# jankammeth/BA-path-planning

Hardware: AMD Instinct MI355X
Metric: SCP iterations/sec (N agents x K waypoints) (higher is better)
Workload: dtype f64

## Files before the change

ba-path-planning_amd/csrc/scp_qp_persist.hip:

```cpp
#include "scp_qp_persist_device.h"

#include <algorithm>
#include <cstdlib>
#include <cerrno>
#include <chrono>


namespace {
using namespace scpdev;
using namespace scp_persist;

#ifdef SCP_PHASE_PROFILE
__device__ unsigned long long scp_persist_clk[16];
#define PSTAMP(slot)                                  \
  do {                                                \
    const unsigned long long now_ = wall_clock64();   \
    pacc[slot] += now_ - plast;                       \
    plast = now_;                                     \
  } while (0)
#else
#define PSTAMP(slot) ((void)0)
#endif

constexpr int persist_apb(int D) { return D == 3 ? 4 : CB / D; }
// ... 580 lines not shown
#pragma unroll
    for (int d = 0; d < D; ++d) {
      const int64_t g = (int64_t)k * C + (int64_t)agent * D + d;
      A.x[g] = x[d];
      A.Qx[g] = qx[d];
    }
  }
  for (int e = threadIdx.x; e < ne; e += NT) {
    A.gval[ebase + e] = e_g[e];
    if (!((e_code[e] >> 16) & 1)) {
      A.zc[e_row[e]] = e_z[e];
      A.yc[e_row[e]] = e_y[e];
      if (with_dy) A.dyc[e_row[e]] = e_pp[(size_t)e * D];
    }
  }
  PSTAMP(8);
#ifdef SCP_PHASE_PROFILE
  if (blockIdx.x == gridDim.x / 2 && threadIdx.x == 0)
    for (int i = 0; i < 16; ++i) scp_persist_clk[i] = i == 15 ? (unsigned long long)steps : pacc[i];
#endif
  if (blockIdx.x == 0 && threadIdx.x == 0) {
    const int slot[NCHK] = {SL_RP, SL_NAX, SL_NZ, SL_RD, SL_NPX, SL_NATY, SL_NDY, SL_SUPP, SL_NATDY};
#pragma unroll
    for (int j = 0; j < NCHK; ++j)
      __hip_atomic_store((u64*)(A.host_scal + slot[j]), (u64)__double_as_longlong(chk[j]), __ATOMIC_RELAXED, __HIP_MEMORY_SCOPE_SYSTEM);
    __hip_atomic_store(A.host_status + 1, (unsigned)it_done, __ATOMIC_RELAXED, __HIP_MEMORY_SCOPE_SYSTEM);
    __hip_atomic_store(A.host_status + 2, n_rho, __ATOMIC_RELAXED, __HIP_MEMORY_SCOPE_SYSTEM);
    __hip_atomic_store((u64*)A.host_rho, (u64)__double_as_longlong(rho), __ATOMIC_RELAXED, __HIP_MEMORY_SCOPE_SYSTEM);
    __hip_atomic_store(A.host_status, exit_code, __ATOMIC_RELAXED, __HIP_MEMORY_SCOPE_SYSTEM);
    __hip_atomic_store(A.host_flag, A.seq, __ATOMIC_RELEASE, __HIP_MEMORY_SCOPE_SYSTEM);
  }
}

size_t persist_lds_bytes(int K, int D, int cap, int nblk) {
  const int apb = persist_apb(D);
  size_t dbl = (size_t)3 * CB * pad_col(K) + (size_t)apb * 64 * D + (size_t)NCHK * nblk + (size_t)cap * (4 * D + 4);
  size_t ints = (size_t)3 * cap + (size_t)apb * K + 1;
  return dbl * sizeof(double) + ((ints + 1) / 2 * 2) * sizeof(int);
}

}

static int persist_variant_for(const scp_qp* qp) {
  const int max_wg = std::min(qp->ctx->n_cu, SCP_PERSIST_MAX_WG);
  const int apb = persist_apb(qp->D);
  const bool fits_old = (qp->N + apb - 1) / apb <= max_wg;
  const bool fits16 = qp->D == 2 && (qp->N + 15) / 16 <= max_wg;
  const bool fits8 = (qp->N + 7) / 8 <= max_wg;
  if (qp->st.persistent == 2 && fits16) return 1;
  if (qp->st.persistent == 3 && fits8) return 2;
  if (qp->st.persistent == 4 && fits_old) return 0;
  if (qp->D == 2) return fits8 ? 2 : (fits16 ? 1 : -1);
  return fits_old ? 0 : (fits8 ? 2 : -1);
}
static int variant_apb(int variant, int D) { return variant == 1 ? 16 : (variant == 2 ? 8 : persist_apb(D)); }

bool scp_qp_persist_eligible(const scp_qp* qp) {
  if (!qp->st.persistent || qp->st.cg_iters != 1 || qp->st.use_mfma != 1) return false;
  if (qp->K > 64 || qp->nW <= 0 || qp->persist_off) return false;
  return persist_variant_for(qp) >= 0;
}

int scp_qp_cg1_persist(scp_qp* qp, int it0, int cad0, int* ran, int* code, int* it_done) {
  const QpDev& d = qp->d;
  scp_ctx* ctx = qp->ctx;
  hipStream_t s = ctx->stream;
  const scp_qp_settings& st = qp->st;
  const int K = qp->K, D = qp->D;
  const int64_t C = qp->C, nx = (int64_t)K * C;
  const int variant = persist_variant_for(qp);
  if (variant < 0) { *ran = 0; return SCP_OK; }
  const bool lean = variant >= 1;
  const int apb = variant_apb(variant, D);
  const int nblk = (qp->N + apb - 1) / apb;
  *ran = 0;
  if (!qp->cg1_ready) {
    int rc = scp_qp_cg1_prepare(qp);
    if (rc) return rc;
  }
  if (qp->persist_cap_nW == qp->nW) return SCP_OK;
  {
    const int nb = nblk + 1;
    const size_t fixed = lean ? scp_persist16_lds_bytes(K, 0, nb, D, apb) : persist_lds_bytes(K, D, 0, nb);
    const size_t per_entry = (size_t)(4 * D + 4) * sizeof(double) + (lean ? 1 : 3) * sizeof(int);
    const size_t budget_lds = 160 * 1024 - (lean ? 2048 : 1024);
    if (fixed + 64 * per_entry > budget_lds) return SCP_OK;
    qp->persist_cap = (int)((budget_lds - fixed) / per_entry / 64 * 64);
  }
  const int nblk_expected = nblk + (qp->persist_fault > 0 ? 1 : 0);
  const size_t lds = lean ? scp_persist16_lds_bytes(K, qp->persist_cap, nblk_expected, D, apb)
                          : persist_lds_bytes(K, D, qp->persist_cap, nblk_expected);
  if (lds > 160 * 1024) return SCP_OK;
  const int budget = st.max_iter - it0;
  if (budget <= 0) return SCP_OK;
  if (!scp_persist_claim(ctx->device, ctx->n_cu, nblk, 200)) {
    qp->persist_skip_solve = true;
    return SCP_OK;
  }
  if (qp->persist_fault > 0) --qp->persist_fault;
  struct ClaimGuard {
    int device, n;
    ~ClaimGuard() { scp_persist_release(device, n); }
  } claim_guard{ctx->device, nblk};
  PersistArgs a;
  a.K = K; a.N = qp->N; a.nblk = nblk_expected; a.ent_cap = qp->persist_cap;
  a.it0 = it0; a.max_iter = st.max_iter; a.check_every = st.check_termination;
  a.cad0 = cad0 > 0 ? cad0 : st.check_termination; a.fine_ratio = st.check_fine_ratio;
  a.check_fine = (st.check_fine > 0 && st.check_fine < st.check_termination && st.check_termination % st.check_fine == 0 && C <= 4096)
                     ? st.check_fine : 0;
  a.rho_interval = st.adaptive_rho_interval > 0 ? st.adaptive_rho_interval : 1;
  a.C = C;
  a.rho = qp->rho; a.rho_c = qp->rho * st.rho_col_scale; a.rho_eq = st.rho_eq_scale; a.alpha = st.alpha; a.h = qp->h;
  a.eps_abs = st.eps_abs; a.eps_rel = st.eps_rel; a.eps_prim_inf = st.eps_prim_inf;
  a.vel_lo = qp->lim[0]; a.vel_hi = qp->lim[1];
  a.acc_lo = qp->lim[2]; a.acc_hi = qp->lim[3]; a.jerk_lo = qp->lim[4]; a.jerk_hi = qp->lim[5];
  for (int dd = 0; dd < 3; ++dd) { a.pmin[dd] = qp->space[dd]; a.pmax[dd] = qp->space[3 + dd]; }
  a.states = d.states;
  a.first_step = qp->steps_since_reset == 0 ? 1 : 0;
  {
    static const int spin_sleep = [] {
      const char* e = getenv("SCP_PERSIST_SPIN_SLEEP");
      const int v = e ? atoi(e) : 1;
      return v < 1 ? 1 : (v > 64 ? 64 : v);
    }();
    a.spin_sleep = spin_sleep;
  }
  a.rho_tol = (st.adaptive_rho && st.adaptive_rho_interval > 0) ? st.adaptive_rho_tolerance : 0.0;
  a.pMinv = d.pMinv;
  a.pT = d.pT;
  a.lf = d.lf; a.uf = d.uf; a.zf = d.zf; a.yf = d.yf; a.fx = d.fx; a.x = d.x;
  a.Qx = qp->qx_sel ? d.HQ : d.HQ + nx;
  a.dyf = d.dyf;
  a.cells = d.cells;
  a.gpart = d.gpart;
  a.gcheck = d.gcheck;
  a.give_up = (unsigned*)d.sync_words;
  a.cell_ptr = d.cell_ptr; a.ent_code = d.ent_code; a.w_k = d.w_k; a.w_i = d.w_i; a.w_j = d.w_j;
  a.w_eta = d.w_eta; a.w_l = d.w_l; a.zc = d.zc; a.yc = d.yc; a.dyc = d.dyc; a.gval = d.gval;
  a.host_status = qp->h_persist_dev;
  a.host_scal = qp->h_scal_dev;
  a.host_flag = (u64*)(qp->h_scal_dev + SL_COUNT + SCP_RESID_CAP);
  a.host_rho = qp->h_scal_dev + SL_COUNT + SCP_RESID_CAP + 3;
  a.rho_col_scale = st.rho_col_scale;
  a.n_tab = 0;
  for (int i = 0; i < qp->n_kkt; ++i)
    if (qp->kkt[i].used && qp->kkt[i].sigma == st.sigma) {
      a.tab[a.n_tab].rho = qp->kkt[i].rho;
      a.tab[a.n_tab].pMinv = qp->kkt[i].pMinv;
      a.tab[a.n_tab].pT = qp->kkt[i].pT;
      ++a.n_tab;
    }
  a.seq = ++qp->check_seq;
  qp->h_persist[0] = 0u;
  qp->h_persist[1] = (unsigned)it0;
  qp->h_persist[2] = 0u;
  qp->persist_rho_switches = 0;
  if (qp->persist_epoch == 0 || qp->persist_epoch + (u64)budget >= 0x7FFFFFF0ull) {
    SCP_HIP_CHECK(ctx, hipMemsetAsync(d.sync_words, 0, 16, s));
    SCP_HIP_CHECK(ctx, hipMemsetAsync(d.cells, 0, (size_t)K * C * 2 * sizeof(u64), s));
    SCP_HIP_CHECK(ctx, hipMemsetAsync(d.gpart, 0, (size_t)SCP_GPART_WORDS * sizeof(u64), s));
    SCP_HIP_CHECK(ctx, hipMemsetAsync(d.gcheck, 0, (size_t)SCP_GCHECK_WORDS * sizeof(u64), s));
    qp->persist_epoch = 0;
  }
  a.epoch0 = (unsigned)qp->persist_epoch;
  qp->persist_variant = variant;
  if (lean) {
    int rc = scp_persist16_launch(ctx, a, nblk, lds, D, apb);
// ... 153 lines not shown
```

ba-path-planning_amd/csrc/scp_qp_persist16.hip:

```cpp
#include "scp_qp_persist_device.h"

namespace {
using namespace scpdev;
using namespace scp_persist;

#ifdef SCP_PHASE_PROFILE
__device__ unsigned long long scp_persist16_clk[16];
#define PSTAMP(slot)                                           \
  do {                                                         \
    if (prof_t) {                                              \
      const unsigned long long now_ = wall_clock64();          \
      pacc_s[slot] += now_ - pacc_s[15];                       \
      pacc_s[15] = now_;                                       \
    }                                                          \
  } while (0)
#else
#define PSTAMP(slot) ((void)0)
#endif

constexpr int nct_of(int D, int APB) { return (D * APB + 15) / 16; }
constexpr int AB_STRIDE = 32;

struct Lds16 {
  int RSK, tK, nks;
  size_t rt, pt, ml, gp, ab, gchk, ent, n_dbl;
  __host__ __device__ Lds16(int K, int cap, int nblk, int D, int APB) {
    const int NC16 = 16 * nct_of(D, APB), APB16 = APB;
    RSK = pad_col(K);
    tK = (K + 15) >> 4;
    nks = (K + 3) >> 2;
    size_t o = 0;
    rt = o; o += (size_t)NC16 * RSK;
    pt = o; o += (size_t)NC16 * RSK;
    ml = o; o += (size_t)tK * nks * 64;
    gp = o; o += (size_t)2 * nblk;
    ab = o; o += (size_t)APB16 * AB_STRIDE;
    if ((size_t)2 * NC16 * RSK >= (size_t)NCHK * nblk) gchk = rt;
    else { gchk = o; o += (size_t)NCHK * nblk; }
    ent = o; o += (size_t)cap * (4 * D + 4);
    n_dbl = o;
  }
};

template <int D, int APB16>
__global__ __launch_bounds__(64 * APB16) void cg1_persist16_kernel(PersistArgs A) {
  constexpr int NT16 = 64 * APB16;
  constexpr int NCT = nct_of(D, APB16);
  constexpr int NC16 = 16 * NCT;
  extern __shared__ __attribute__((aligned(16))) double lds[];
  __shared__ double red[NCHK][APB16];
  __shared__ double cert_s[3][APB16];
  __shared__ double chk_s[NCHK];
  __shared__ int fail_s;
#ifdef SCP_PHASE_PROFILE
  __shared__ unsigned long long pacc_s[16];
  const bool prof_t = blockIdx.x == gridDim.x / 2 && threadIdx.x == 0;
  if (prof_t) {
    for (int i = 0; i < 15; ++i) pacc_s[i] = 0;
    pacc_s[15] = wall_clock64();
  }
#endif
  const int K = A.K, N = A.N;
  const int64_t C = A.C;
  const int cap = A.ent_cap, nblk = A.nblk;
  const Lds16 L(K, cap, nblk, D, APB16);
  const int RSK = L.RSK, tK = L.tK, nks = L.nks;
  double* Rt = lds + L.rt;
  double* Pt = lds + L.pt;
  double* Ml = lds + L.ml;
  double* gp = lds + L.gp;
  double* ab = lds + L.ab;
  double* gck = lds + L.gchk;
  double* e_c = lds + L.ent;
  double* e_l = e_c + (size_t)cap * D;
  double* e_z = e_l + cap;
  double* e_y = e_z + cap;
  double* e_g = e_y + cap;
  double* e_qo = e_g + cap;
  double* e_qp = e_qo + (size_t)cap * D;
  double* e_pp = e_qp + (size_t)cap * D;
  int* e_code = (int*)(lds + L.n_dbl);
  int* cptr = e_code + cap;

  const int wave = threadIdx.x >> 6, lane = threadIdx.x & 63;
  const int a0 = blockIdx.x * APB16;
  const int agent = a0 + wave;
  const bool aok = agent < N;
  const int k = lane;
  const bool live = aok && k < K;
  const bool jok = live && k < K - 1;
  const bool lastk = k == K - 1;
  const double h = A.h, hh = h * h, ih = 1.0 / h, alpha = A.alpha;
  double rho = A.rho, rho_c = A.rho_c;
  unsigned n_rho = 0;

  const int a1 = min(a0 + APB16, N);
  const int ebase = A.cell_ptr[cell_of(0, a0, K)];
  const int ne = A.cell_ptr[cell_of(0, a1, K)] - ebase;
  {
    int worst = 0;
    for (int b = threadIdx.x; b < (N + APB16 - 1) / APB16; b += NT16) {
      const int b0 = b * APB16, b1 = min(b0 + APB16, N);
      worst = max(worst, A.cell_ptr[cell_of(0, b1, K)] - A.cell_ptr[cell_of(0, b0, K)]);
    }
    if (__syncthreads_or(worst > cap)) {
      if (blockIdx.x == 0 && threadIdx.x == 0) {
        __hip_atomic_store(A.host_status, (unsigned)EXIT_OVERFLOW, __ATOMIC_RELAXED, __HIP_MEMORY_SCOPE_SYSTEM);
        __hip_atomic_store(A.host_flag, A.seq, __ATOMIC_RELEASE, __HIP_MEMORY_SCOPE_SYSTEM);
      }
      return;
    }
  }
  if (threadIdx.x == 0) fail_s = 0;
  for (int i = threadIdx.x; i <= (a1 - a0) * K; i += NT16) cptr[i] = A.cell_ptr[cell_of(0, a0, K) + i] - ebase;
  for (int e = threadIdx.x; e < ne; e += NT16) {
    const int code = A.ent_code[ebase + e];
    const int n = code >> 1, side = code & 1;
    const int wi = A.w_i[n], wj = A.w_j[n], wk = A.w_k[n];
    const int own = side ? wj : wi, par = side ? wi : wj;
    e_code[e] = wk | ((own - a0) << 6) | (side << 10) | (par << 11);
    const int64_t bo = (int64_t)wk * C + (int64_t)own * D, bp = (int64_t)wk * C + (int64_t)par * D;
#pragma unroll
    for (int d = 0; d < D; ++d) {
      const double eta = A.w_eta[(size_t)n * D + d];
      e_c[(size_t)e * D + d] = side ? -eta : eta;
      e_qo[(size_t)e * D + d] = A.Qx[bo + d];
      e_qp[(size_t)e * D + d] = A.Qx[bp + d];
    }
    e_l[e] = A.w_l[n];
    e_z[e] = A.zc[n];
    e_y[e] = A.yc[n];
    e_g[e] = A.gval[ebase + e];
  }
  for (int i = threadIdx.x; i < NC16 * RSK; i += NT16) Rt[i] = 0.0;
  for (int i = threadIdx.x; i < tK * nks * 64; i += NT16) Ml[i] = A.pMinv[i];

  double v[D][4], off[D], x[D], c1[D], c2[D];
#pragma unroll
  for (int t = 0; t < 4; ++t) {
    const bool rok = t == 0 ? jok : live;
    const int row = t == 0 ? k : t * K - 1 + k;
    const double rr = (t >= 2 && lastk) ? rho * A.rho_eq : rho;
#pragma unroll
    for (int d = 0; d < D; ++d) {
      v[d][t] = 0.0;
      if (rok) {
        const int64_t g = (int64_t)row * C + (int64_t)agent * D + d;
        v[d][t] = A.zf[g] + A.yf[g] / rr;
      }
    }
  }
  if (threadIdx.x < APB16 * D) {
    const int al = threadIdx.x / D, d = threadIdx.x % D, ag = a0 + al;
    double* o = ab + al * AB_STRIDE;
    const bool there = ag < N;
    const double v0 = there ? A.states[((size_t)N + ag) * D + d] : 0.0;
    o[d] = A.vel_lo - v0;
    o[4 + d] = A.vel_hi - v0;
    o[8 + d] = (there ? A.states[((size_t)3 * N + ag) * D + d] : 0.0) - v0;
    o[12 + d] = A.pmin[d];
    o[16 + d] = A.pmax[d];
    o[20 + d] = there ? A.states[((size_t)2 * N + ag) * D + d] : 0.0;
    o[24 + d] = -1e300;
    o[28 + d] = 1e300;
  }
#pragma unroll
  for (int d = 0; d < D; ++d) {
#pragma clang fp contract(off)
    const double p0 = aok ? A.states[(size_t)agent * D + d] : 0.0, v0 = aok ? A.states[((size_t)N + agent) * D + d] : 0.0;
    const double hk = h * (double)(k + 1);
    const double hkv = hk * v0;
    off[d] = p0 + hkv;
  }
  const double* const tb = ab + wave * AB_STRIDE;
  const double* const b_vl = tb + (live ? (lastk ? 8 : 0) : 24);
  const double* const b_vh = tb + (live ? (lastk ? 8 : 4) : 28);
  const double* const b_pl = tb + (live ? (lastk ? 20 : 12) : 24);
  const double* const b_ph = tb + (live ? (lastk ? 20 : 16) : 28);
  auto bounds = [&](int d, double (&lo)[2], double (&hi)[2]) {
    lo[0] = b_vl[d];
    hi[0] = b_vh[d];
    lo[1] = b_pl[d] - off[d];
    hi[1] = b_ph[d] - off[d];
  };
#pragma unroll
  for (int d = 0; d < D; ++d) {
    x[d] = live ? A.x[(int64_t)k * C + (int64_t)agent * D + d] : 0.0;
    const double s1 = wave_incl_sum(x[d]);
    const double s2 = lane_below(wave_incl_sum(s1));
    c1[d] = live ? s1 : 0.0;
    c2[d] = live ? s2 : 0.0;
  }
  const double jlo = A.jerk_lo, jhi = A.jerk_hi, alo = A.acc_lo, ahi = A.acc_hi;
  __syncthreads();
  const int c0 = aok ? cptr[wave * K + min(k, K - 1)] : 0;
  const int c1e = (aok && k < K) ? cptr[wave * K + k + 1] : c0;
  const bool has_rows = c1e > c0;
  u64* my_cell = A.cells + ((size_t)((int64_t)min(k, K - 1) * N + (aok ? agent : 0)) * D) * 2;
  double* my_pt = Pt + (size_t)(wave * D) * RSK + k;
  double* my_rt = Rt + (size_t)(wave * D) * RSK + k;

  PSTAMP(0);
  bool ok = true;
  int it_done = A.it0;
  unsigned steps = 0;
  unsigned exit_code = 0;
  const bool with_dy = A.eps_prim_inf > 0.0;
  if (threadIdx.x < 3 * APB16) (&cert_s[0][0])[threadIdx.x] = 0.0;
  int cad = A.cad0;
  for (;;) {
  int nit = cad - it_done % cad;
  if (it_done + nit > A.max_iter) nit = A.max_iter - it_done;
  for (int it = 0; it < nit; ++it, ++steps) {
    const unsigned tag = A.epoch0 + steps + 1u;
    const bool last = it == nit - 1;
    const bool first = A.first_step && steps == 0u;
    u64* gpart = A.gpart + (size_t)(tag & 1u) * nblk * 4;
    const double rv = lastk ? rho * A.rho_eq : rho;
    {
      double r[D];
      double g[D];
#pragma unroll
      for (int d = 0; d < D; ++d) g[d] = 0.0;
      for (int e = c0; e < c1e; ++e) {
        const double ge = e_g[e];
#pragma unroll
        for (int d = 0; d < D; ++d) g[d] += e_c[(size_t)e * D + d] * ge;
      }
#pragma unroll
      for (int d = 0; d < D; ++d) {
        double lo[2], hi[2];
        bounds(d, lo, hi);
        const double xn = lane_above(x[d]);
        double cj = fmin(fmax(v[d][0], jlo), jhi), ca = fmin(fmax(v[d][1], alo), ahi);
        double cv = fmin(fmax(v[d][2], lo[0]), hi[0]), cp = fmin(fmax(v[d][3], lo[1]), hi[1]);
        if (first) { cj = v[d][0]; ca = v[d][1]; cv = v[d][2]; cp = v[d][3]; }
        const double wj = jok ? rho * ((cj - (xn - x[d]) * ih) - (v[d][0] - cj)) : 0.0;
        const double wa = rho * ((ca - x[d]) - (v[d][1] - ca));
        const double wv = rv * ((cv - h * c1[d]) - (v[d][2] - cv));
        const double wp = rv * ((cp - hh * (c2[d] + 0.5 * c1[d])) - (v[d][3] - cp));
        const double u1 = h * wv + 0.5 * hh * (wp - g[d]);
        const double u2 = wp + g[d];
        const double d1 = wave_incl_rsum(u1);
        const double s1 = wave_incl_rsum(u2);
        const double d2 = lane_above(wave_incl_rsum(s1));
        const double wjm = lane_below(wj);
        r[d] = (((wjm - wj) * ih + wa) + (d1 + 0.5 * hh * g[d]) + hh * d2) - 2.0 * x[d];
        if (live) my_rt[d * RSK] = r[d];
        __builtin_amdgcn_sched_barrier(0);
      }
    }
    __syncthreads();
    PSTAMP(1);
    if (wave < 4 * NCT && (wave & 3) < tK) {
      const int li = lane & 15, lk = lane >> 4;
      const int tile = wave & 3, ct = wave >> 2;
      const double* Mt = Ml + (size_t)tile * nks * 64 + lane;
      const double* Bt = Rt + (size_t)(ct * 16 + li) * RSK;
      double4_t acc = {0.0, 0.0, 0.0, 0.0};
#pragma unroll 4
      for (int s = 0; s < nks; ++s) {
        const int kk = 4 * s + lk;
        const double b = kk < K ? Bt[kk] : 0.0;
        acc = __builtin_amdgcn_mfma_f64_16x16x4f64(Mt[(size_t)s * 64], b, acc, 0, 0, 0);
      }
      double* Ot = Pt + (size_t)(ct * 16 + li) * RSK;
#pragma unroll
      for (int q = 0; q < 4; ++q) {
        const int row = tile * 16 + lk + 4 * q;
        if (row < K) Ot[row] = acc[q];
      }
    }
    __syncthreads();
    PSTAMP(2);
    double p[D], s1p[D], s2p[D];
    {
      double rz = 0.0;
#pragma unroll
      for (int d = 0; d < D; ++d) {
        p[d] = live ? my_pt[d * RSK] : 0.0;
        rz += (live ? my_rt[d * RSK] : 0.0) * p[d];
        const double cs1 = wave_incl_sum(p[d]);
        const double cs2 = lane_below(wave_incl_sum(cs1));
        const double qp = hh * (cs2 - 0.5 * lane_below(cs1));
        s1p[d] = live ? cs1 : 0.0;
        s2p[d] = live ? cs2 : 0.0;
        if (has_rows) {
          st_granules(my_cell + 2 * d, tag, qp);
          my_pt[d * RSK] = qp;
        }
      }
      rz = wave_incl_sum(rz);
      if (lane == 63) red[0][wave] = rz;
    }
    __syncthreads();
    PSTAMP(3);
    {
      double sq = 0.0;
      unsigned spins = 0;
      bool bad = false;
      for (int e = threadIdx.x; e < ne; e += NT16) {
        const int code = e_code[e];
        const int ek = code & 63, al = (code >> 6) & 15, side = (code >> 10) & 1, par = code >> 11;
        const u64* pc = A.cells + ((size_t)((int64_t)ek * N + par) * D) * 2;
        u32x4 w[D];
        for (;;) {
          ld_cell<D>(pc, w);
          bool here = true;
#pragma unroll
          for (int d = 0; d < D; ++d) here = here && pair_ok(w[d], tag);
          if (here) break;
          if (++spins > SPIN_LIMIT || ((spins & 255u) == 0u &&
                                       __hip_atomic_load(A.give_up, __ATOMIC_RELAXED, __HIP_MEMORY_SCOPE_AGENT) != 0u)) {
            bad = true;
            break;
          }
          spin_nap(A.spin_sleep);
        }
        if (bad) break;
        double s = 0.0;
#pragma unroll
        for (int d = 0; d < D; ++d) {
          const double pp = pair_value(w[d]);
          e_pp[(size_t)e * D + d] = pp;
          s += e_c[(size_t)e * D + d] * (Pt[(size_t)(al * D + d) * RSK + ek] - pp);
        }
        if (!side) sq += s * s;
      }
      if (bad) {
        __hip_atomic_store(A.give_up, 1u, __ATOMIC_RELAXED, __HIP_MEMORY_SCOPE_AGENT);
        fail_s = 1;
      }
      sq = wave_incl_sum(sq);
      if (lane == 63) red[1][wave] = sq;
    }
    __syncthreads();
    if (fail_s) { ok = false; break; }
    PSTAMP(4);
    if (threadIdx.x < 2) {
      double t = 0.0;
#pragma unroll
      for (int w = 0; w < APB16; ++w) t += red[threadIdx.x][w];
      st_granules(gpart + (size_t)blockIdx.x * 4 + 2 * threadIdx.x, tag, t);
    }
    {
      unsigned spins = 0;
      bool bad = false;
      for (int q = threadIdx.x; q < 2 * nblk; q += NT16) {
        u32x4 w;
        for (;;) {
          w = ld_pair(gpart + 2 * q);
          if (pair_ok(w, tag)) break;
          if (++spins > SPIN_LIMIT || ((spins & 255u) == 0u &&
                                       __hip_atomic_load(A.give_up, __ATOMIC_RELAXED, __HIP_MEMORY_SCOPE_AGENT) != 0u)) {
            bad = true;
            break;
          }
          spin_nap(A.spin_sleep);
        }
        if (bad) break;
        gp[q] = pair_value(w);
      }
      if (bad) {
        __hip_atomic_store(A.give_up, 1u, __ATOMIC_RELAXED, __HIP_MEMORY_SCOPE_AGENT);
        fail_s = 1;
      }
    }
    __syncthreads();
    if (fail_s) { ok = false; break; }
    PSTAMP(5);
    double a;
    {
      double vr = 0.0, vs = 0.0;
      for (int b = lane; b < nblk; b += 64) {
        vr += gp[2 * b];
        vs += gp[2 * b + 1];
      }
      const double rzt = read_lane(wave_incl_sum(vr), 63);
      const double sqt = read_lane(wave_incl_sum(vs), 63);
      const double pHp = rzt + rho_c * sqt;
      a = (pHp > 0.0 && rzt != 0.0) ? rzt / pHp : 0.0;
    }
    const double aa = alpha * a;
    PSTAMP(6);
    {
      const double irc = 1.0 / rho_c;
      for (int e = threadIdx.x; e < ne; e += NT16) {
        const int code = e_code[e];
        const int ek = code & 63, al = (code >> 6) & 15;
        double tc = 0.0, ax = 0.0;
#pragma unroll
        for (int d = 0; d < D; ++d) {
          const double c = e_c[(size_t)e * D + d];
          const double po = Pt[(size_t)(al * D + d) * RSK + ek], pp = e_pp[(size_t)e * D + d];
          const double qo = e_qo[(size_t)e * D + d], qq = e_qp[(size_t)e * D + d];
          tc += c * (fma(a, po, qo) - fma(a, pp, qq));
          const double qon = fma(aa, po, qo), qqn = fma(aa, pp, qq);
          ax += c * (qon - qqn);
          e_qo[(size_t)e * D + d] = qon;
          e_qp[(size_t)e * D + d] = qqn;
        }
        const double zo = e_z[e], yo = e_y[e];
        const double zh = alpha * tc + (1.0 - alpha) * zo;
        const double zn = fmax(zh + yo * irc, e_l[e]);
        const double yn = yo + rho_c * (zh - zn);
        e_z[e] = zn;
        e_y[e] = yn;
        e_g[e] = (rho_c * zn - yn) - rho_c * ax;
        if (last && with_dy) e_pp[(size_t)e * D] = fmin(yn - yo, 0.0);
      }
    }
    const bool cert = last && with_dy;
    if (cert) __syncthreads();
    double m_ndy = 0.0, m_supp = 0.0, m_natdy = 0.0;
    {
#pragma unroll
      for (int d = 0; d < D; ++d) {
        const double xt = fma(a, p[d], x[d]);
        const double t1 = fma(a, s1p[d], c1[d]), t2 = fma(a, s2p[d], c2[d]);
        const double xtn = lane_above(xt);
        double lo[2], hi[2];
        bounds(d, lo, hi);
        double cj = fmin(fmax(v[d][0], jlo), jhi), ca = fmin(fmax(v[d][1], alo), ahi);
        double cv = fmin(fmax(v[d][2], lo[0]), hi[0]), cp = fmin(fmax(v[d][3], lo[1]), hi[1]);
        if (first) { cj = v[d][0]; ca = v[d][1]; cv = v[d][2]; cp = v[d][3]; }
        const double nj = jok ? fma(alpha, (xtn - xt) * ih - cj, v[d][0]) : v[d][0];
        const double na = fma(alpha, xt - ca, v[d][1]);
        const double nv = fma(alpha, h * t1 - cv, v[d][2]);
        const double np = fma(alpha, hh * (t2 + 0.5 * t1) - cp, v[d][3]);
        if (cert) {
          const double dyj = rho * ((nj - fmin(fmax(nj, jlo), jhi)) - (v[d][0] - cj));
          const double dya = rho * ((na - fmin(fmax(na, alo), ahi)) - (v[d][1] - ca));
          const double dyv = rv * ((nv - fmin(fmax(nv, lo[0]), hi[0])) - (v[d][2] - cv));
          const double dyp = rv * ((np - fmin(fmax(np, lo[1]), hi[1])) - (v[d][3] - cp));
          m_ndy = fmax(m_ndy, fmax(fmax(fabs(dyj), fabs(dya)), fmax(fabs(dyv), fabs(dyp))));
          m_supp += (jhi * fmax(dyj, 0.0) + jlo * fmin(dyj, 0.0)) + (ahi * fmax(dya, 0.0) + alo * fmin(dya, 0.0)) +
                    (hi[0] * fmax(dyv, 0.0) + lo[0] * fmin(dyv, 0.0)) + (hi[1] * fmax(dyp, 0.0) + lo[1] * fmin(dyp, 0.0));
          double gd = 0.0;
          for (int e = c0; e < c1e; ++e) gd += e_c[(size_t)e * D + d] * e_pp[(size_t)e * D];
          const double u1 = h * dyv + 0.5 * hh * (dyp - gd);
          const double u2 = dyp + gd;
          const double d1 = wave_incl_rsum(u1);
          const double s1 = wave_incl_rsum(u2);
          const double d2 = lane_above(wave_incl_rsum(s1));
          const double vjm = lane_below(dyj);
          const double at = ((vjm - dyj) * ih + dya) + (d1 + 0.5 * hh * gd) + hh * d2;
          if (live) m_natdy = fmax(m_natdy, fabs(at));
        }
        v[d][0] = nj; v[d][1] = na; v[d][2] = nv; v[d][3] = np;
        x[d] = fma(aa, p[d], x[d]);
        c1[d] = fma(aa, s1p[d], c1[d]);
        c2[d] = fma(aa, s2p[d], c2[d]);
        __builtin_amdgcn_sched_barrier(0);
      }
    }
    if (cert) {
      m_ndy = wave_max_nn(m_ndy);
      m_supp = wave_incl_sum(m_supp);
      m_natdy = wave_max_nn(m_natdy);
      if (lane == 63) { cert_s[0][wave] = m_ndy; cert_s[1][wave] = m_supp; cert_s[2][wave] = m_natdy; }
    }
    __syncthreads();
    PSTAMP(7);
  }

  if (!ok) break;
  it_done += nit;
  {
    const unsigned ctag = 0x80000000u | (A.epoch0 + steps);
    const double rv = lastk ? rho * A.rho_eq : rho;
    double m[NCHK];
#pragma unroll
    for (int j = 0; j < NCHK; ++j) m[j] = 0.0;
    {
      double gy[D];
#pragma unroll
      for (int d = 0; d < D; ++d) gy[d] = 0.0;
      for (int e = c0; e < c1e; ++e) {
        const double ye = e_y[e];
#pragma unroll
        for (int d = 0; d < D; ++d) gy[d] += e_c[(size_t)e * D + d] * ye;
      }
#pragma unroll
      for (int d = 0; d < D; ++d) {
        const double s1 = wave_incl_sum(x[d]);
        const double s2 = lane_below(wave_incl_sum(s1));
        const double qx = hh * (s2 - 0.5 * lane_below(s1));
        c1[d] = live ? s1 : 0.0;
        c2[d] = live ? s2 : 0.0;
        if (has_rows) {
          st_granules(my_cell + 2 * d, ctag, qx);
          my_pt[d * RSK] = qx;
        }
        double lo[2], hi[2];
        bounds(d, lo, hi);
        const double xn = lane_above(x[d]);
        const double f[4] = {jok ? (xn - x[d]) * ih : 0.0, x[d], h * c1[d], hh * (c2[d] + 0.5 * c1[d])};
        const double zc[4] = {fmin(fmax(v[d][0], jlo), jhi), fmin(fmax(v[d][1], alo), ahi),
                              fmin(fmax(v[d][2], lo[0]), hi[0]), fmin(fmax(v[d][3], lo[1]), hi[1])};
#pragma unroll
        for (int t = 0; t < 4; ++t) {
          if (t == 0 ? jok : live) {
            m[CK_RP] = fmax(m[CK_RP], fabs(f[t] - zc[t]));
            m[CK_NAX] = fmax(m[CK_NAX], fabs(f[t]));
            m[CK_NZ] = fmax(m[CK_NZ], fabs(zc[t]));
          }
        }
        const double vj = jok ? rho * (v[d][0] - zc[0]) : 0.0, va = rho * (v[d][1] - zc[1]);
        const double vv = rv * (v[d][2] - zc[2]), vp = rv * (v[d][3] - zc[3]);
        const double g = gy[d];
        const double u1 = h * vv + 0.5 * hh * (vp - g);
        const double u2 = vp + g;
        const double d1 = wave_incl_rsum(u1);
        const double r1 = wave_incl_rsum(u2);
        const double d2 = lane_above(wave_incl_rsum(r1));
        const double vjm = lane_below(vj);
        const double at = ((vjm - vj) * ih + va) + (d1 + 0.5 * hh * g) + hh * d2;
        if (live) {
          const double px = 2.0 * x[d];
          m[CK_RD] = fmax(m[CK_RD], fabs(px + at));
          m[CK_NPX] = fmax(m[CK_NPX], fabs(px));
          m[CK_NATY] = fmax(m[CK_NATY], fabs(at));
        }
        __builtin_amdgcn_sched_barrier(0);
      }
    }
    __syncthreads();
    {
      unsigned spins = 0;
      bool bad = false;
      for (int e = threadIdx.x; e < ne; e += NT16) {
        const int code = e_code[e];
        const int ek = code & 63, al = (code >> 6) & 15, side = (code >> 10) & 1, par = code >> 11;
        const u64* pc = A.cells + ((size_t)((int64_t)ek * N + par) * D) * 2;
        u32x4 w[D];
        for (;;) {
          ld_cell<D>(pc, w);
          bool here = true;
#pragma unroll
          for (int d = 0; d < D; ++d) here = here && pair_ok(w[d], ctag);
          if (here) break;
          if (++spins > SPIN_LIMIT || ((spins & 255u) == 0u &&
                                       __hip_atomic_load(A.give_up, __ATOMIC_RELAXED, __HIP_MEMORY_SCOPE_AGENT) != 0u)) {
            bad = true;
            break;
          }
          spin_nap(A.spin_sleep);
        }
        if (bad) break;
        double ax = 0.0;
#pragma unroll
        for (int d = 0; d < D; ++d) {
          const double qq = pair_value(w[d]);
          const double qo = Pt[(size_t)(al * D + d) * RSK + ek];
          e_qo[(size_t)e * D + d] = qo;
          e_qp[(size_t)e * D + d] = qq;
          ax += e_c[(size_t)e * D + d] * (qo - qq);
        }
        if (!side) {
          const double zc_ = e_z[e];
          m[CK_RP] = fmax(m[CK_RP], fabs(ax - zc_));
          m[CK_NAX] = fmax(m[CK_NAX], fabs(ax));
          m[CK_NZ] = fmax(m[CK_NZ], fabs(zc_));
          if (with_dy) {
            const double dd = e_pp[(size_t)e * D];
            m[CK_NDY] = fmax(m[CK_NDY], fabs(dd));
            m[CK_SUPP] += e_l[e] * dd;
          }
        }
      }
      if (bad) {
        __hip_atomic_store(A.give_up, 1u, __ATOMIC_RELAXED, __HIP_MEMORY_SCOPE_AGENT);
        fail_s = 1;
      }
    }
#pragma unroll
    for (int j = 0; j < NCHK; ++j) {
      double v = j == CK_SUPP ? wave_incl_sum(m[j]) : wave_max_nn(m[j]);
      if (lane == 63) {
        if (j == CK_NDY) v = fmax(v, cert_s[0][wave]);
        if (j == CK_SUPP) v += cert_s[1][wave];
        if (j == CK_NATDY) v = fmax(v, cert_s[2][wave]);
        red[j][wave] = v;
      }
    }
    __syncthreads();
    if (fail_s) { ok = false; break; }
    if (threadIdx.x < NCHK) {
      double t = 0.0;
#pragma unroll
      for (int w = 0; w < APB16; ++w) t = threadIdx.x == CK_SUPP ? t + red[threadIdx.x][w] : fmax(t, red[threadIdx.x][w]);
      st_granules(A.gcheck + ((size_t)blockIdx.x * NCHK + threadIdx.x) * 2, ctag, t);
    }
    {
      unsigned spins = 0;
      bool bad = false;
      for (int q = threadIdx.x; q < NCHK * nblk; q += NT16) {
        u32x4 w;
        for (;;) {
          w = ld_pair(A.gcheck + 2 * q);
          if (pair_ok(w, ctag)) break;
          if (++spins > SPIN_LIMIT || ((spins & 255u) == 0u &&
                                       __hip_atomic_load(A.give_up, __ATOMIC_RELAXED, __HIP_MEMORY_SCOPE_AGENT) != 0u)) {
            bad = true;
            break;
          }
          spin_nap(A.spin_sleep);
        }
        if (bad) break;
        gck[q] = pair_value(w);
      }
      if (bad) {
        __hip_atomic_store(A.give_up, 1u, __ATOMIC_RELAXED, __HIP_MEMORY_SCOPE_AGENT);
        fail_s = 1;
      }
    }
    __syncthreads();
    if (fail_s) { ok = false; break; }
    double chk[NCHK];
#pragma unroll
    for (int j = 0; j < NCHK; ++j) {
      double v = 0.0;
      for (int b = lane; b < nblk; b += 64) v = j == CK_SUPP ? v + gck[b * NCHK + j] : fmax(v, gck[b * NCHK + j]);
      chk[j] = read_lane(j == CK_SUPP ? wave_incl_sum(v) : wave_max_nn(v), 63);
    }
    if (threadIdx.x == 0) {
#pragma unroll
      for (int j = 0; j < NCHK; ++j) chk_s[j] = chk[j];
    }
    __syncthreads();
    if (L.gchk == L.rt) {
      for (int i = threadIdx.x; i < NC16 * RSK; i += NT16) Rt[i] = 0.0;
    }
    const double np_ = fmax(chk[CK_NAX], chk[CK_NZ]), nd_ = fmax(chk[CK_NPX], chk[CK_NATY]);
    const double tol_p = A.eps_abs + A.eps_rel * np_, tol_d = A.eps_abs + A.eps_rel * nd_;
    if (chk[CK_RP] <= tol_p && chk[CK_RD] <= tol_d) { exit_code = EXIT_SOLVED; break; }
    if (A.check_fine > 0)
      cad = (chk[CK_RP] < A.fine_ratio * tol_p && chk[CK_RD] < A.fine_ratio * tol_d) ? A.check_fine : A.check_every;
    if (it_done >= A.max_iter) { exit_code = EXIT_MAX_ITER; break; }
    if (with_dy && chk[CK_NDY] > A.eps_prim_inf && chk[CK_SUPP] < -A.eps_prim_inf * chk[CK_NDY] &&
        chk[CK_NATDY] < A.eps_prim_inf * chk[CK_NDY]) { exit_code = EXIT_INFEASIBLE; break; }
    if (A.rho_tol > 0.0 && it_done % A.rho_interval == 0) {
      const double prim = chk[CK_RP] / fmax(np_, 1e-10), dual = chk[CK_RD] / fmax(nd_, 1e-10);
      const double nr = fmin(fmax(rho * sqrt(prim / fmax(dual, 1e-10)), 1e-6), 1e6);
      const double cand = exp2(round(4.0 * log2(nr)) * 0.25);
      if (cand > rho * A.rho_tol * (1.0 - 1e-9) || cand < rho / A.rho_tol * (1.0 + 1e-9)) {
        int slot = -1;
        for (int i = 0; i < A.n_tab; ++i)
          if (fabs(A.tab[i].rho - cand) <= 1e-12 * cand) slot = i;
        if (slot < 0) { exit_code = EXIT_RHO; break; }
        const double nrs = A.tab[slot].rho;
        if (nrs > rho * A.rho_tol || nrs < rho / A.rho_tol) {
          {
#pragma unroll
            for (int d = 0; d < D; ++d) {
              double lo[2], hi[2];
              bounds(d, lo, hi);
              const double zc[4] = {fmin(fmax(v[d][0], jlo), jhi), fmin(fmax(v[d][1], alo), ahi),
                                    fmin(fmax(v[d][2], lo[0]), hi[0]), fmin(fmax(v[d][3], lo[1]), hi[1])};
#pragma unroll
              for (int t = 0; t < 4; ++t) {
                const double rr_old = (t >= 2 && lastk) ? rho * A.rho_eq : rho, rr_new = (t >= 2 && lastk) ? nrs * A.rho_eq : nrs;
                const double yv = rr_old * (v[d][t] - zc[t]);
                v[d][t] = zc[t] + yv / rr_new;
              }
            }
          }
          rho = nrs;
          rho_c = rho * A.rho_col_scale;
          for (int i = threadIdx.x; i < tK * nks * 64; i += NT16) Ml[i] = A.tab[slot].pMinv[i];
          for (int e = threadIdx.x; e < ne; e += NT16) {
            double ax = 0.0;
#pragma unroll
            for (int d = 0; d < D; ++d) ax += e_c[(size_t)e * D + d] * (e_qo[(size_t)e * D + d] - e_qp[(size_t)e * D + d]);
            e_g[e] = (rho_c * e_z[e] - e_y[e]) - rho_c * ax;
          }
          ++n_rho;
          if (A.check_fine > 0) cad = A.check_fine;
        }
      }
    }
    __syncthreads();
    PSTAMP(9);
  }
  }

  if (ok && __syncthreads_or(threadIdx.x == 0 &&
                             __hip_atomic_load(A.give_up, __ATOMIC_RELAXED, __HIP_MEMORY_SCOPE_AGENT) != 0u))
    ok = false;
  if (!ok) {
    if (threadIdx.x == 0) {
      __hip_atomic_store(A.host_status, (unsigned)EXIT_GAVE_UP, __ATOMIC_RELAXED, __HIP_MEMORY_SCOPE_SYSTEM);
      __hip_atomic_store(A.host_flag, A.seq, __ATOMIC_RELEASE, __HIP_MEMORY_SCOPE_SYSTEM);
    }
    return;
  }
#pragma unroll
  for (int d = 0; d < D; ++d) {
    const double xn = lane_above(x[d]);
    const double c1b = lane_below(c1[d]);
    double lo[2], hi[2];
    bounds(d, lo, hi);
    const double f[4] = {(xn - x[d]) * ih, x[d], h * c1[d], hh * (c2[d] + 0.5 * c1[d])};
    const double zc[4] = {fmin(fmax(v[d][0], jlo), jhi), fmin(fmax(v[d][1], alo), ahi),
                          fmin(fmax(v[d][2], lo[0]), hi[0]), fmin(fmax(v[d][3], lo[1]), hi[1])};
#pragma unroll
    for (int t = 0; t < 4; ++t) {
      if (t == 0 ? jok : live) {
        const int row = t == 0 ? k : t * K - 1 + k;
        const int64_t g = (int64_t)row * C + (int64_t)agent * D + d;
        A.zf[g] = zc[t];
        A.yf[g] = ((t >= 2 && lastk) ? rho * A.rho_eq : rho) * (v[d][t] - zc[t]);
        A.fx[g] = f[t];
      }
    }
    if (live) {
      const int64_t g = (int64_t)k * C + (int64_t)agent * D + d;
      A.x[g] = x[d];
      A.Qx[g] = hh * (c2[d] - 0.5 * c1b);
    }
  }
  for (int e = threadIdx.x; e < ne; e += NT16) {
    A.gval[ebase + e] = e_g[e];
    if (!((e_code[e] >> 10) & 1)) {
      const int n = A.ent_code[ebase + e] >> 1;
      A.zc[n] = e_z[e];
      A.yc[n] = e_y[e];
    }
  }
  PSTAMP(8);
#ifdef SCP_PHASE_PROFILE
  if (prof_t)
    for (int i = 0; i < 16; ++i) scp_persist16_clk[i] = i == 15 ? (unsigned long long)steps : pacc_s[i];
#endif
  if (blockIdx.x == 0 && threadIdx.x == 0) {
    const int slot[NCHK] = {SL_RP, SL_NAX, SL_NZ, SL_RD, SL_NPX, SL_NATY, SL_NDY, SL_SUPP, SL_NATDY};
#pragma unroll
    for (int j = 0; j < NCHK; ++j)
      __hip_atomic_store((u64*)(A.host_scal + slot[j]), (u64)__double_as_longlong(chk_s[j]), __ATOMIC_RELAXED, __HIP_MEMORY_SCOPE_SYSTEM);
    __hip_atomic_store(A.host_status + 1, (unsigned)it_done, __ATOMIC_RELAXED, __HIP_MEMORY_SCOPE_SYSTEM);
    __hip_atomic_store(A.host_status + 2, n_rho, __ATOMIC_RELAXED, __HIP_MEMORY_SCOPE_SYSTEM);
    __hip_atomic_store((u64*)A.host_rho, (u64)__double_as_longlong(rho), __ATOMIC_RELAXED, __HIP_MEMORY_SCOPE_SYSTEM);
    __hip_atomic_store(A.host_status, exit_code, __ATOMIC_RELAXED, __HIP_MEMORY_SCOPE_SYSTEM);
    __hip_atomic_store(A.host_flag, A.seq, __ATOMIC_RELEASE, __HIP_MEMORY_SCOPE_SYSTEM);
  }
}

}

#ifdef SCP_PHASE_PROFILE
extern "C" int scp_debug_persist16_clocks(unsigned long long* out, int n) {
  if (n > 16) n = 16;
  return hipMemcpyFromSymbol(out, HIP_SYMBOL(scp_persist16_clk), (size_t)n * sizeof(unsigned long long)) == hipSuccess ? 0 : 1;
}
#endif

size_t scp_persist16_lds_bytes(int K, int cap, int nblk, int D, int apb) {
  const Lds16 L(K, cap, nblk, D, apb);
  const size_t ints = (size_t)cap + (size_t)apb * K + 1;
  return L.n_dbl * sizeof(double) + ((ints + 1) / 2 * 2) * sizeof(int);
}

template <int D, int APB>
static int launch16(scp_ctx* ctx, const PersistArgs& a, int nblk, size_t lds) {
  if (lds > 64 * 1024)
    SCP_HIP_CHECK(ctx, scp_raise_lds_limit(ctx->device, reinterpret_cast<const void*>(cg1_persist16_kernel<D, APB>), lds));
  hipLaunchKernelGGL((cg1_persist16_kernel<D, APB>), dim3(nblk), dim3(64 * APB), lds, ctx->stream, a);
  SCP_HIP_CHECK(ctx, hipGetLastError());
  return SCP_OK;
}

int scp_persist16_launch(scp_ctx* ctx, const PersistArgs& a, int nblk, size_t lds, int D, int apb) {
  if (D == 2 && apb == 16) return launch16<2, 16>(ctx, a, nblk, lds);
  if (D == 2 && apb == 8) return launch16<2, 8>(ctx, a, nblk, lds);
  if (D == 3 && apb == 8) return launch16<3, 8>(ctx, a, nblk, lds);
  return scp_fail(ctx, SCP_ERR_INVALID, "persistent kernel: no instantiation for D = %d with %d agents per workgroup", D, apb);
}
```

ba-path-planning_amd/csrc/scp_qp_persist_device.h:

```cpp
#pragma once
#include "scp_qp_device.h"

namespace scp_persist {
using namespace scpdev;

typedef unsigned long long u64;
constexpr unsigned SPIN_LIMIT = 1u << 20;

struct PersistArgs {
  int K, N, nblk, ent_cap;
  int it0, max_iter, check_every, rho_interval;
  int cad0, check_fine;
  double fine_ratio;
  int64_t C;
  double rho, rho_c, rho_eq, alpha, h;
  double eps_abs, eps_rel, eps_prim_inf, rho_tol;
  double jerk_lo, jerk_hi, acc_lo, acc_hi, vel_lo, vel_hi, pmin[3], pmax[3];
  const double* states;
  int first_step;
  int spin_sleep;
  const double* pMinv;
  const double* pT;
  const double *lf, *uf;
  double *zf, *yf, *fx, *x, *Qx, *dyf;
  u64* cells;
  u64* gpart;
  u64* gcheck;
  unsigned* give_up;
  const int *cell_ptr, *ent_code, *w_k, *w_i, *w_j;
  const double *w_eta, *w_l;
  double *zc, *yc, *dyc, *gval;
  unsigned* host_status;
  double* host_scal;
  u64* host_flag;
  u64 seq;
  unsigned epoch0;
  double rho_col_scale;
  double* host_rho;
  int n_tab;
  struct RhoSlot {
    double rho;
    const double* pMinv;
    const double* pT;
  } tab[SCP_KKT_SLOTS_MAX];
};

enum { EXIT_SOLVED = 1, EXIT_GAVE_UP = 2, EXIT_MAX_ITER = 3, EXIT_INFEASIBLE = 4, EXIT_RHO = 5, EXIT_OVERFLOW = 6 };
constexpr int NCHK = 9;
constexpr int CK_RP = 0, CK_NAX = 1, CK_NZ = 2, CK_RD = 3, CK_NPX = 4, CK_NATY = 5, CK_NDY = 6, CK_SUPP = 7, CK_NATDY = 8;

typedef unsigned int u32x4 __attribute__((ext_vector_type(4)));
__device__ inline void st_granules(u64* g, unsigned tag, double v) {
  const u32x4 w = {(unsigned)__double2loint(v), tag, (unsigned)__double2hiint(v), tag};
  asm volatile("global_store_dwordx4 %0, %1, off sc1" ::"v"(g), "v"(w) : "memory");
}
__device__ inline u32x4 ld_pair(const u64* g) {
  u32x4 w;
  asm volatile("global_load_dwordx4 %0, %1, off sc1\n\ts_waitcnt vmcnt(0)" : "=v"(w) : "v"(g) : "memory");
  return w;
}
template <int D>
__device__ inline void ld_cell(const u64* g, u32x4 (&w)[D]) {
  if (D == 2) {
    asm volatile("global_load_dwordx4 %0, %2, off sc1\n\tglobal_load_dwordx4 %1, %2, off offset:16 sc1\n\ts_waitcnt vmcnt(0)"
                 : "=&v"(w[0]), "=&v"(w[1])
                 : "v"(g)
                 : "memory");
  } else {
#pragma unroll
    for (int d = 0; d < D; ++d) w[d] = ld_pair(g + 2 * d);
  }
}
__device__ inline void spin_nap(int n) {
  for (int i = 0; i < n; ++i) __builtin_amdgcn_s_sleep(1);
}
__device__ inline bool pair_ok(const u32x4& w, unsigned tag) { return w[1] == tag && w[3] == tag; }
__device__ inline double pair_value(const u32x4& w) { return __hiloint2double((int)w[2], (int)w[0]); }


}

size_t scp_persist16_lds_bytes(int K, int cap, int nblk, int D, int apb);
int scp_persist16_launch(scp_ctx* ctx, const scp_persist::PersistArgs& a, int nblk, size_t lds, int D, int apb);
```

Before: 385.0.

## Compress collision entry state to scalar projections and compute Q-transform via MFMA

Each collision entry now holds the scalar projections ax and s in LDS instead of per-dimension Qx copies of both agents. This shrinks entry storage from 4D+4 to D+6 doubles, which raises entry capacity and cuts per-iteration LDS traffic in the z/y update. For small D*APB configurations, the lean kernel computes the transformed direction with extra MFMA waves using a cached pT matrix, instead of scan-based cumulative sums, and removes one block barrier on that path. It also hoists the constraint clamp computation ahead of the spin wait. The cost is extra LDS for the Qt and Tl buffers and a reliance on algebraic identities being exact in f64.

```diff
diff --git a/ba-path-planning_amd/csrc/scp_qp_persist.hip b/ba-path-planning_amd/csrc/scp_qp_persist.hip
--- a/ba-path-planning_amd/csrc/scp_qp_persist.hip
+++ b/ba-path-planning_amd/csrc/scp_qp_persist.hip
@@ -686,7 +686,7 @@
   {
     const int nb = nblk + 1;
     const size_t fixed = lean ? scp_persist16_lds_bytes(K, 0, nb, D, apb) : persist_lds_bytes(K, D, 0, nb);
-    const size_t per_entry = (size_t)(4 * D + 4) * sizeof(double) + (lean ? 1 : 3) * sizeof(int);
+    const size_t per_entry = lean ? scp_persist16_entry_bytes(D) : (size_t)(4 * D + 4) * sizeof(double) + 3 * sizeof(int);
     const size_t budget_lds = 160 * 1024 - (lean ? 2048 : 1024);
     if (fixed + 64 * per_entry > budget_lds) return SCP_OK;
     qp->persist_cap = (int)((budget_lds - fixed) / per_entry / 64 * 64);
diff --git a/ba-path-planning_amd/csrc/scp_qp_persist16.hip b/ba-path-planning_amd/csrc/scp_qp_persist16.hip
--- a/ba-path-planning_amd/csrc/scp_qp_persist16.hip
+++ b/ba-path-planning_amd/csrc/scp_qp_persist16.hip
@@ -21,11 +21,15 @@
 constexpr int nct_of(int D, int APB) { return (D * APB + 15) / 16; }
 constexpr int AB_STRIDE = 32;
 
+constexpr bool t_on_mfma(int D, int APB) { return 4 * nct_of(D, APB) < APB && APB <= 8; }
+constexpr int ent_doubles(int D) { return D + 6; }
+
 struct Lds16 {
   int RSK, tK, nks;
-  size_t rt, pt, ml, gp, ab, gchk, ent, n_dbl;
+  size_t rt, pt, qt, ml, tl, gp, ab, gchk, ent, n_dbl;
   __host__ __device__ Lds16(int K, int cap, int nblk, int D, int APB) {
     const int NC16 = 16 * nct_of(D, APB), APB16 = APB;
+    const bool tq = t_on_mfma(D, APB);
     RSK = pad_col(K);
     tK = (K + 15) >> 4;
     nks = (K + 3) >> 2;
@@ -33,11 +37,17 @@
     rt = o; o += (size_t)NC16 * RSK;
     pt = o; o += (size_t)NC16 * RSK;
     ml = o; o += (size_t)tK * nks * 64;
+    qt = pt;
+    tl = ml;
+    if (tq) {
+      qt = o; o += (size_t)NC16 * RSK;
+      tl = o; o += (size_t)tK * nks * 64;
+    }
     gp = o; o += (size_t)2 * nblk;
     ab = o; o += (size_t)APB16 * AB_STRIDE;
     if ((size_t)2 * NC16 * RSK >= (size_t)NCHK * nblk) gchk = rt;
     else { gchk = o; o += (size_t)NCHK * nblk; }
-    ent = o; o += (size_t)cap * (4 * D + 4);
+    ent = o; o += (size_t)cap * ent_doubles(D);
     n_dbl = o;
   }
 };
@@ -47,6 +57,7 @@
   constexpr int NT16 = 64 * APB16;
   constexpr int NCT = nct_of(D, APB16);
   constexpr int NC16 = 16 * NCT;
+  constexpr bool TQ = t_on_mfma(D, APB16);
   extern __shared__ __attribute__((aligned(16))) double lds[];
   __shared__ double red[NCHK][APB16];
   __shared__ double cert_s[3][APB16];
@@ -67,7 +78,9 @@
   const int RSK = L.RSK, tK = L.tK, nks = L.nks;
   double* Rt = lds + L.rt;
   double* Pt = lds + L.pt;
+  double* Qt = lds + L.qt;
   double* Ml = lds + L.ml;
+  double* Tl = lds + L.tl;
   double* gp = lds + L.gp;
   double* ab = lds + L.ab;
   double* gck = lds + L.gchk;
@@ -76,9 +89,8 @@
   double* e_z = e_l + cap;
   double* e_y = e_z + cap;
   double* e_g = e_y + cap;
-  double* e_qo = e_g + cap;
-  double* e_qp = e_qo + (size_t)cap * D;
-  double* e_pp = e_qp + (size_t)cap * D;
+  double* e_ax = e_g + cap;
+  double* e_s = e_ax + cap;
   int* e_code = (int*)(lds + L.n_dbl);
   int* cptr = e_code + cap;
 
@@ -120,20 +132,25 @@
     const int own = side ? wj : wi, par = side ? wi : wj;
     e_code[e] = wk | ((own - a0) << 6) | (side << 10) | (par << 11);
     const int64_t bo = (int64_t)wk * C + (int64_t)own * D, bp = (int64_t)wk * C + (int64_t)par * D;
+    double ax = 0.0;
 #pragma unroll
     for (int d = 0; d < D; ++d) {
       const double eta = A.w_eta[(size_t)n * D + d];
-      e_c[(size_t)e * D + d] = side ? -eta : eta;
-      e_qo[(size_t)e * D + d] = A.Qx[bo + d];
-      e_qp[(size_t)e * D + d] = A.Qx[bp + d];
-    }
+      const double c = side ? -eta : eta;
+      e_c[(size_t)e * D + d] = c;
+      ax += c * (A.Qx[bo + d] - A.Qx[bp + d]);
+    }
+    e_ax[e] = ax;
     e_l[e] = A.w_l[n];
     e_z[e] = A.zc[n];
     e_y[e] = A.yc[n];
     e_g[e] = A.gval[ebase + e];
   }
   for (int i = threadIdx.x; i < NC16 * RSK; i += NT16) Rt[i] = 0.0;
-  for (int i = threadIdx.x; i < tK * nks * 64; i += NT16) Ml[i] = A.pMinv[i];
+  for (int i = threadIdx.x; i < tK * nks * 64; i += NT16) {
+    Ml[i] = A.pMinv[i];
+    if constexpr (TQ) Tl[i] = A.pT[i];
+  }
 
   double v[D][4], off[D], x[D], c1[D], c2[D];
 #pragma unroll
@@ -252,10 +269,11 @@
     }
     __syncthreads();
     PSTAMP(1);
-    if (wave < 4 * NCT && (wave & 3) < tK) {
+    if ((wave < 4 * NCT || (TQ && wave < 4 * NCT + 4)) && (wave & 3) < tK) {
+      const bool tw = TQ && wave >= 4 * NCT;
       const int li = lane & 15, lk = lane >> 4;
-      const int tile = wave & 3, ct = wave >> 2;
-      const double* Mt = Ml + (size_t)tile * nks * 64 + lane;
+      const int tile = wave & 3, ct = tw ? 0 : wave >> 2;
+      const double* Mt = (tw ? Tl : Ml) + (size_t)tile * nks * 64 + lane;
       const double* Bt = Rt + (size_t)(ct * 16 + li) * RSK;
       double4_t acc = {0.0, 0.0, 0.0, 0.0};
 #pragma unroll 4
@@ -264,11 +282,26 @@
         const double b = kk < K ? Bt[kk] : 0.0;
         acc = __builtin_amdgcn_mfma_f64_16x16x4f64(Mt[(size_t)s * 64], b, acc, 0, 0, 0);
       }
-      double* Ot = Pt + (size_t)(ct * 16 + li) * RSK;
-#pragma unroll
-      for (int q = 0; q < 4; ++q) {
-        const int row = tile * 16 + lk + 4 * q;
-        if (row < K) Ot[row] = acc[q];
+      if (TQ && tw) {
+        const int al = li / D, d = li % D;
+        const bool col_ok = li < D * APB16 && a0 + al < N;
+        double* Ot = Qt + (size_t)li * RSK;
+#pragma unroll
+        for (int q = 0; q < 4; ++q) {
+          const int row = tile * 16 + lk + 4 * q;
+          if (row < K) {
+            Ot[row] = acc[q];
+            if (col_ok && cptr[al * K + row + 1] > cptr[al * K + row])
+              st_granules(A.cells + ((size_t)((int64_t)row * N + a0 + al) * D + d) * 2, tag, acc[q]);
+          }
+        }
+      } else {
+        double* Ot = Pt + (size_t)(ct * 16 + li) * RSK;
+#pragma unroll
+        for (int q = 0; q < 4; ++q) {
+          const int row = tile * 16 + lk + 4 * q;
+          if (row < K) Ot[row] = acc[q];
+        }
       }
     }
     __syncthreads();
@@ -282,18 +315,20 @@
         rz += (live ? my_rt[d * RSK] : 0.0) * p[d];
         const double cs1 = wave_incl_sum(p[d]);
         const double cs2 = lane_below(wave_incl_sum(cs1));
-        const double qp = hh * (cs2 - 0.5 * lane_below(cs1));
         s1p[d] = live ? cs1 : 0.0;
         s2p[d] = live ? cs2 : 0.0;
-        if (has_rows) {
-          st_granules(my_cell + 2 * d, tag, qp);
-          my_pt[d * RSK] = qp;
+        if constexpr (!TQ) {
+          const double qp = hh * (cs2 - 0.5 * lane_below(cs1));
+          if (has_rows) {
+            st_granules(my_cell + 2 * d, tag, qp);
+            my_pt[d * RSK] = qp;
+          }
         }
       }
       rz = wave_incl_sum(rz);
       if (lane == 63) red[0][wave] = rz;
     }
-    __syncthreads();
+    if constexpr (!TQ) __syncthreads();
     PSTAMP(3);
     {
       double sq = 0.0;
@@ -320,11 +355,8 @@
         if (bad) break;
         double s = 0.0;
 #pragma unroll
-        for (int d = 0; d < D; ++d) {
-          const double pp = pair_value(w[d]);
-          e_pp[(size_t)e * D + d] = pp;
-          s += e_c[(size_t)e * D + d] * (Pt[(size_t)(al * D + d) * RSK + ek] - pp);
-        }
+        for (int d = 0; d < D; ++d) s += e_c[(size_t)e * D + d] * (Qt[(size_t)(al * D + d) * RSK + ek] - pair_value(w[d]));
+        e_s[e] = s;
         if (!side) sq += s * s;
       }
       if (bad) {
@@ -342,6 +374,20 @@
 #pragma unroll
       for (int w = 0; w < APB16; ++w) t += red[threadIdx.x][w];
       st_granules(gpart + (size_t)blockIdx.x * 4 + 2 * threadIdx.x, tag, t);
+    }
+    double zcl[D][4];
+#pragma unroll
+    for (int d = 0; d < D; ++d) {
+      double lo[2], hi[2];
+      bounds(d, lo, hi);
+      zcl[d][0] = fmin(fmax(v[d][0], jlo), jhi);
+      zcl[d][1] = fmin(fmax(v[d][1], alo), ahi);
+      zcl[d][2] = fmin(fmax(v[d][2], lo[0]), hi[0]);
+      zcl[d][3] = fmin(fmax(v[d][3], lo[1]), hi[1]);
+      if (first) {
+#pragma unroll
+        for (int t = 0; t < 4; ++t) zcl[d][t] = v[d][t];
+      }
     }
     {
       unsigned spins = 0;
@@ -386,20 +432,9 @@
     {
       const double irc = 1.0 / rho_c;
       for (int e = threadIdx.x; e < ne; e += NT16) {
-        const int code = e_code[e];
-        const int ek = code & 63, al = (code >> 6) & 15;
-        double tc = 0.0, ax = 0.0;
-#pragma unroll
-        for (int d = 0; d < D; ++d) {
-          const double c = e_c[(size_t)e * D + d];
-          const double po = Pt[(size_t)(al * D + d) * RSK + ek], pp = e_pp[(size_t)e * D + d];
-          const double qo = e_qo[(size_t)e * D + d], qq = e_qp[(size_t)e * D + d];
-          tc += c * (fma(a, po, qo) - fma(a, pp, qq));
-          const double qon = fma(aa, po, qo), qqn = fma(aa, pp, qq);
-          ax += c * (qon - qqn);
-          e_qo[(size_t)e * D + d] = qon;
-          e_qp[(size_t)e * D + d] = qqn;
-        }
+        const double s = e_s[e], ax0 = e_ax[e];
+        const double tc = fma(a, s, ax0), ax = fma(aa, s, ax0);
+        e_ax[e] = ax;
         const double zo = e_z[e], yo = e_y[e];
         const double zh = alpha * tc + (1.0 - alpha) * zo;
         const double zn = fmax(zh + yo * irc, e_l[e]);
@@ -407,7 +442,7 @@
         e_z[e] = zn;
         e_y[e] = yn;
         e_g[e] = (rho_c * zn - yn) - rho_c * ax;
-        if (last && with_dy) e_pp[(size_t)e * D] = fmin(yn - yo, 0.0);
+        if (last && with_dy) e_s[e] = fmin(yn - yo, 0.0);
       }
     }
     const bool cert = last && with_dy;
@@ -419,16 +454,14 @@
         const double xt = fma(a, p[d], x[d]);
         const double t1 = fma(a, s1p[d], c1[d]), t2 = fma(a, s2p[d], c2[d]);
         const double xtn = lane_above(xt);
-        double lo[2], hi[2];
-        bounds(d, lo, hi);
-        double cj = fmin(fmax(v[d][0], jlo), jhi), ca = fmin(fmax(v[d][1], alo), ahi);
-        double cv = fmin(fmax(v[d][2], lo[0]), hi[0]), cp = fmin(fmax(v[d][3], lo[1]), hi[1]);
-        if (first) { cj = v[d][0]; ca = v[d][1]; cv = v[d][2]; cp = v[d][3]; }
+        const double cj = zcl[d][0], ca = zcl[d][1], cv = zcl[d][2], cp = zcl[d][3];
         const double nj = jok ? fma(alpha, (xtn - xt) * ih - cj, v[d][0]) : v[d][0];
         const double na = fma(alpha, xt - ca, v[d][1]);
         const double nv = fma(alpha, h * t1 - cv, v[d][2]);
         const double np = fma(alpha, hh * (t2 + 0.5 * t1) - cp, v[d][3]);
         if (cert) {
+          double lo[2], hi[2];
+          bounds(d, lo, hi);
           const double dyj = rho * ((nj - fmin(fmax(nj, jlo), jhi)) - (v[d][0] - cj));
           const double dya = rho * ((na - fmin(fmax(na, alo), ahi)) - (v[d][1] - ca));
           const double dyv = rv * ((nv - fmin(fmax(nv, lo[0]), hi[0])) - (v[d][2] - cv));
@@ -437,7 +470,7 @@
           m_supp += (jhi * fmax(dyj, 0.0) + jlo * fmin(dyj, 0.0)) + (ahi * fmax(dya, 0.0) + alo * fmin(dya, 0.0)) +
                     (hi[0] * fmax(dyv, 0.0) + lo[0] * fmin(dyv, 0.0)) + (hi[1] * fmax(dyp, 0.0) + lo[1] * fmin(dyp, 0.0));
           double gd = 0.0;
-          for (int e = c0; e < c1e; ++e) gd += e_c[(size_t)e * D + d] * e_pp[(size_t)e * D];
+          for (int e = c0; e < c1e; ++e) gd += e_c[(size_t)e * D + d] * e_s[e];
           const double u1 = h * dyv + 0.5 * hh * (dyp - gd);
           const double u2 = dyp + gd;
           const double d1 = wave_incl_rsum(u1);
@@ -553,17 +586,16 @@
         for (int d = 0; d < D; ++d) {
           const double qq = pair_value(w[d]);
           const double qo = Pt[(size_t)(al * D + d) * RSK + ek];
-          e_qo[(size_t)e * D + d] = qo;
-          e_qp[(size_t)e * D + d] = qq;
           ax += e_c[(size_t)e * D + d] * (qo - qq);
         }
+        e_ax[e] = ax;
         if (!side) {
           const double zc_ = e_z[e];
           m[CK_RP] = fmax(m[CK_RP], fabs(ax - zc_));
           m[CK_NAX] = fmax(m[CK_NAX], fabs(ax));
           m[CK_NZ] = fmax(m[CK_NZ], fabs(zc_));
           if (with_dy) {
-            const double dd = e_pp[(size_t)e * D];
+            const double dd = e_s[e];
             m[CK_NDY] = fmax(m[CK_NDY], fabs(dd));
             m[CK_SUPP] += e_l[e] * dd;
           }
@@ -668,13 +700,12 @@
           }
           rho = nrs;
           rho_c = rho * A.rho_col_scale;
-          for (int i = threadIdx.x; i < tK * nks * 64; i += NT16) Ml[i] = A.tab[slot].pMinv[i];
-          for (int e = threadIdx.x; e < ne; e += NT16) {
-            double ax = 0.0;
-#pragma unroll
-            for (int d = 0; d < D; ++d) ax += e_c[(size_t)e * D + d] * (e_qo[(size_t)e * D + d] - e_qp[(size_t)e * D + d]);
-            e_g[e] = (rho_c * e_z[e] - e_y[e]) - rho_c * ax;
-          }
+          for (int i = threadIdx.x; i < tK * nks * 64; i += NT16) {
+            Ml[i] = A.tab[slot].pMinv[i];
+            if constexpr (TQ) Tl[i] = A.tab[slot].pT[i];
+          }
+          for (int e = threadIdx.x; e < ne; e += NT16)
+            e_g[e] = (rho_c * e_z[e] - e_y[e]) - rho_c * e_ax[e];
           ++n_rho;
           if (A.check_fine > 0) cad = A.check_fine;
         }
@@ -755,6 +786,8 @@
 }
 #endif
 
+size_t scp_persist16_entry_bytes(int D) { return (size_t)ent_doubles(D) * sizeof(double) + sizeof(int); }
+
 size_t scp_persist16_lds_bytes(int K, int cap, int nblk, int D, int apb) {
   const Lds16 L(K, cap, nblk, D, apb);
   const size_t ints = (size_t)cap + (size_t)apb * K + 1;
diff --git a/ba-path-planning_amd/csrc/scp_qp_persist_device.h b/ba-path-planning_amd/csrc/scp_qp_persist_device.h
--- a/ba-path-planning_amd/csrc/scp_qp_persist_device.h
+++ b/ba-path-planning_amd/csrc/scp_qp_persist_device.h
@@ -81,4 +81,5 @@
 }
 
 size_t scp_persist16_lds_bytes(int K, int cap, int nblk, int D, int apb);
+size_t scp_persist16_entry_bytes(int D);
 int scp_persist16_launch(scp_ctx* ctx, const scp_persist::PersistArgs& a, int nblk, size_t lds, int D, int apb);
```

Result: faster. 417.3 (median of 6 runs) (+8.4%).
